# omerkurt-okt/buck-gnn

Measured on NVIDIA B200. Metric: graphs/sec, higher is better.
Workload: dtype f16

## Files before the change

buckgnn_b200/capi.py:

```python
from __future__ import annotations

import ctypes as C
import os
import threading

from .build import LIB_PATH as _DEFAULT_LIB_PATH

LIB_PATH = os.environ.get("BG_LIB_PATH", _DEFAULT_LIB_PATH)

BG_BF16, BG_F32, BG_F16 = 0, 1, 2
BG_AGGR_MEAN, BG_AGGR_SUM, BG_AGGR_MAX = 0, 1, 2
BG_BIG_ROW_THRESHOLD = 64
BG_MAX_GEMM_SEGMENTS = 8
ABI_VERSION = 11

AGGR_CODES = {"mean": BG_AGGR_MEAN, "sum": BG_AGGR_SUM, "add": BG_AGGR_SUM, "max": BG_AGGR_MAX}

EXPORTED_SYMBOLS = (
    "bg_abi_version", "bg_last_error", "bg_device_check", "bg_watchdog_info_host", "bg_set_sm_partition",
    "bg_csr_max_big_rows", "bg_csr_workspace_bytes", "bg_csr_build",
    "bg_batch_info", "bg_graph_ptr_build", "bg_publish_words", "bg_encoder_front",
    "bg_aggregate_workspace_bytes", "bg_hubfold_workspace_bytes", "bg_sage_aggregate", "bg_gemm512",
    "bg_sage_fused512", "bg_sage_aggregate_hubs", "bg_gemm128", "bg_gemm128_gathered", "bg_pool_head128", "bg_pool_head_blocks128",
    "bg_wgrad512", "bg_pool_workspace_bytes", "bg_pool_head", "bg_pool_block_flags", "bg_pool_head_blocks", "bg_cast_f32", "bg_split_tf32",
    "bg_expand_rowptr", "bg_add",
    "bg_train_workspace_bytes", "bg_bn_batch_stats", "bg_bn_act_forward", "bg_sage_backward_rows",
    "bg_transpose_chunks", "bg_mask_narrow", "bg_reduce_partials", "bg_colsum_workspace_bytes", "bg_colsum", "bg_pool_backward",
    "bg_sgemm_workspace_bytes", "bg_sgemm", "bg_eigen_loss", "bg_dropout_mask", "bg_collate_ptr", "bg_collate", "bg_expand_wire",
    "bg_dropout_residual", "bg_grad_mask", "bg_segment_expand",
    "bg_sag_workspace_bytes", "bg_sag_select", "bg_sag_connect", "bg_gather_rows", "bg_index_invert", "bg_index_gather",
    "bg_sag_pool_backward", "bg_max_aggregate_backward", "bg_max_bwd_workspace_bytes",
    "bg_bn_batch_stats128", "bg_bn_act_forward128", "bg_sage_backward_rows128", "bg_pool_backward128",
    "bg_max_aggregate_backward128", "bg_wgrad128",
    "bg_dropout_residual128", "bg_grad_mask128", "bg_segment_expand128", "bg_wgrad128_ld",
)


class BuckGNNError(RuntimeError):
    def __init__(self, status: int, where: str, message: str):
        super().__init__(f"{where} failed with status {status}: {message}")
        self.status = status


class GemmSegment(C.Structure):
    _fields_ = [("a", C.c_void_p), ("lda", C.c_int64), ("b", C.c_void_p), ("ldb", C.c_int64),
                ("k", C.c_int32), ("b_groups", C.c_int32)]


class Epilogue(C.Structure):
    _fields_ = [("bias_host", C.c_void_p), ("bn_scale_host", C.c_void_p), ("bn_shift_host", C.c_void_p),
                ("residual", C.c_void_p), ("ldr", C.c_int64), ("normalize", C.c_int32), ("relu", C.c_int32),
                ("gather", C.c_void_p * 2),
                ("gather_idx", C.c_void_p * 2), ("gather_ld", C.c_int64), ("inv_norm_out", C.c_void_p),
                ("pool_block_sums", C.c_void_p), ("pool_block_keep", C.c_void_p)]


class FusedAggregate(C.Structure):
    _fields_ = [("x", C.c_void_p), ("ldx", C.c_int64), ("rowptr", C.c_void_p), ("col", C.c_void_p),
                ("aggr", C.c_int32), ("n_big", C.c_int32), ("hub_agg", C.c_void_p), ("big_rows", C.c_void_p)]


_lib = None
_lock = threading.Lock()
_P, _I64, _I32, _SZP = C.c_void_p, C.c_int64, C.c_int32, C.POINTER(C.c_size_t)

_SIGNATURES = {
    "bg_abi_version": (C.c_int, []),
    "bg_last_error": (C.c_char_p, []),
    "bg_device_check": (C.c_int, []),
    "bg_watchdog_info_host": (C.c_int, [C.POINTER(C.c_uint32)]),
    "bg_set_sm_partition": (C.c_int, [C.c_int, C.c_int]),
    "bg_csr_max_big_rows": (_I64, [_I64]),
    "bg_csr_workspace_bytes": (C.c_int, [_I64, _I64, _SZP]),
    "bg_csr_build": (C.c_int, [_P, _I64, _I64, C.c_int, _P, _P, _P, _P, _P, _P, _P, _P, C.c_size_t, _P]),
    "bg_batch_info": (C.c_int, [_P, _I64, _P, _P]),
    "bg_publish_words": (C.c_int, [_P, _P, _I32, _P]),
    "bg_graph_ptr_build": (C.c_int, [_P, _I64, _I64, _P, _P]),
    "bg_encoder_front": (C.c_int, [_P, _I64, _I32, _P, _P, _P, _P, _P, _P, C.c_int, _P, _P]),
    "bg_expand_rowptr": (C.c_int, [_P, _I64, _I64, _P, _P, _P, C.c_int, C.c_int, _P]),
    "bg_add": (C.c_int, [_P, _P, _P, _P, C.c_int, _I64, _P]),
    "bg_aggregate_workspace_bytes": (C.c_int, [_I32, _SZP]),
    "bg_hubfold_workspace_bytes": (C.c_int, [_I64, C.c_int, _I32, _I32, _SZP]),
    "bg_sage_aggregate": (C.c_int, [_P, _P, C.c_int, _I64, _I32, _P, _P, _P, _I32, C.c_int, _P, _P, _I32, _P,
                                    C.c_size_t, _P]),
    "bg_gemm512": (C.c_int, [C.POINTER(GemmSegment), _I32, _I64, C.c_int, C.c_int, C.POINTER(Epilogue), _P,
                             C.c_int, _I64, C.c_int, _P]),
    "bg_sage_fused512": (C.c_int, [C.POINTER(GemmSegment), _I32, _I64, C.c_int, C.c_int, C.POINTER(Epilogue),
                                   C.POINTER(FusedAggregate), _P, C.c_int, _I64, _P]),
    "bg_sage_aggregate_hubs": (C.c_int, [_P, C.c_int, _P, _P, _P, _I32, C.c_int, _P, _P, C.c_size_t, _P]),
    "bg_gemm128": (C.c_int, [C.POINTER(GemmSegment), _I32, _I64, C.c_int, C.c_int, C.POINTER(Epilogue), _P,
                             C.c_int, _I64, C.c_int, _P]),
    "bg_gemm128_gathered": (C.c_int, [C.POINTER(GemmSegment), _I32, _I64, C.c_int, C.c_int, C.POINTER(Epilogue), _P,
                                      C.c_int, _I64, C.c_int, _P]),
    "bg_pool_head128": (C.c_int, [_P, C.c_int, _I64, _P, _I64, C.c_int, _P, _P, _P, _P, _P, _P, _P, _P, _I32, _P, _P,
                                  _P, C.c_size_t, _P, _P]),
    "bg_pool_head_blocks128": (C.c_int, [_P, C.c_int, _I64, _P, _I64, C.c_int, _P, _P, _P, _P, _P, _P, _P, _P, _I32, _P,
                                         _P, _P, _P, _P, C.c_size_t, _P, _P]),
    "bg_wgrad512": (C.c_int, [_P, _I64, _P, _I32, _I64, C.c_int, _I64, _I32, _I64, _P, _P]),
    "bg_pool_workspace_bytes": (C.c_int, [_I64, _SZP]),
    "bg_pool_head": (C.c_int, [_P, C.c_int, _I64, _P, _I64, C.c_int, _P, _P, _P, _P, _P, _P, _P, _P, _I32, _P, _P,
                               _P, C.c_size_t, _P, _P]),
    "bg_pool_block_flags": (C.c_int, [_P, _I64, _I64, _P, _P]),
    "bg_pool_head_blocks": (C.c_int, [_P, C.c_int, _I64, _P, _I64, C.c_int, _P, _P, _P, _P, _P, _P, _P, _P, _I32, _P, _P,
                                      _P, _P, _P, C.c_size_t, _P, _P]),
    "bg_cast_f32": (C.c_int, [_P, _P, C.c_int, _I64, _P]),
    "bg_split_tf32": (C.c_int, [_P, _P, _P, _I64, _P]),
    "bg_train_workspace_bytes": (C.c_int, [_I64, _SZP]),
# ... 84 lines not shown
    buf = (C.c_uint32 * 4)()
    _check(load().bg_watchdog_info_host(buf), "bg_watchdog_info_host")
    return list(buf)


def csr_max_big_rows(n_edges: int) -> int:
    return int(load().bg_csr_max_big_rows(n_edges))


def _query(fn_name: str, *args) -> int:
    out = C.c_size_t(0)
    _check(getattr(load(), fn_name)(*args, C.byref(out)), fn_name)
    return int(out.value)


def csr_workspace_bytes(n_nodes: int, n_edges: int) -> int:
    return _query("bg_csr_workspace_bytes", n_nodes, n_edges)


def aggregate_workspace_bytes(n_big: int) -> int:
    return _query("bg_aggregate_workspace_bytes", n_big)


def pool_workspace_bytes(n_graphs: int) -> int:
    return _query("bg_pool_workspace_bytes", n_graphs)


def csr_build(edge_index, n_edges, n_nodes, key_row, rowptr, col, perm, big_rows, info, ws, ws_bytes, stream,
              hub_lo=None, hub_of_row=None):
    _check(load().bg_csr_build(edge_index, n_edges, n_nodes, key_row, rowptr, col, perm, big_rows, info,
                               hub_lo, hub_of_row, ws, ws_bytes, stream), "bg_csr_build")


def batch_info(batch, n_nodes, info, stream):
    _check(load().bg_batch_info(batch, n_nodes, info, stream), "bg_batch_info")


def publish_words(src, dst_host_mapped, n, stream):
    _check(load().bg_publish_words(src, dst_host_mapped, n, stream), "bg_publish_words")


def graph_ptr_build(batch, n_nodes, n_graphs, graph_ptr, stream):
    _check(load().bg_graph_ptr_build(batch, n_nodes, n_graphs, graph_ptr, stream), "bg_graph_ptr_build")


def encoder_front(x, n_nodes, n_features, w1, b1, w2, b2, out, out_dtype, stream, row_gather=None, nonfinite=None):
    _check(load().bg_encoder_front(x, n_nodes, n_features, w1, b1, w2, b2, row_gather, out, out_dtype, nonfinite, stream),
           "bg_encoder_front")


def expand_rowptr(rowptr, n_rows, n_entries, row_of, iota, nonempty, nonempty_dtype, stream, as_count=False):
    _check(load().bg_expand_rowptr(rowptr, n_rows, n_entries, row_of, iota, nonempty, nonempty_dtype,
                                   int(bool(as_count)), stream), "bg_expand_rowptr")


def add(a, b, c, out, dtype, n, stream):
    _check(load().bg_add(a, b, c, out, dtype, n, stream), "bg_add")


def hubfold_workspace_bytes(n_nodes: int, dtype: int, n_big: int, hub_max_degree: int) -> int:
    return _query("bg_hubfold_workspace_bytes", n_nodes, dtype, n_big, hub_max_degree)


def sage_aggregate(x, out, dtype, n_nodes, rowptr, col, big_rows, n_big, aggr, ws, ws_bytes, stream, width=512,
                   hub_lo=None, hub_of_row=None, hub_max_degree=0):
    _check(load().bg_sage_aggregate(x, out, dtype, n_nodes, width, rowptr, col, big_rows, n_big, aggr,
# ... 267 lines not shown
```

buckgnn_b200/csrc/capi.cu:

```cuda
#include <cstdio>
#include <cstring>

#include "common.cuh"
#include "csr_build.cuh"
#include "aggregate.cuh"
#include "aggregate_window.cuh"
#include "encoder.cuh"
#include "gemm_tc.cuh"
#include "gemm128.cuh"
#include "pool_head.cuh"
#include "train.cuh"
#include "sag_pool.cuh"
#include "max_bwd.cuh"

namespace bg {

static thread_local char g_last_error[512] = "";

void set_last_cuda_error(cudaError_t e, const char* what, const char* file, int line) {
  snprintf(g_last_error, sizeof(g_last_error), "CUDA error %d (%s) at %s:%d: %s", (int)e,
           cudaGetErrorString(e), file, line, what);
}
static int fail(int code, const char* msg) {
  snprintf(g_last_error, sizeof(g_last_error), "%s", msg);
// ... 332 lines not shown
  const int max_big = (int)bg_csr_max_big_rows(E);
  const int sms = sm_count();
  BG_CUDA_OK(cudaMemsetAsync(w.deg, 0, sizeof(int32_t) * (size_t)(N + 1), stream));
  if ((hub_lo != nullptr) != (hub_of_row != nullptr)) return fail(BG_ERR_INVALID, "bg_csr_build: hub_lo and hub_of_row go together");
  BG_CUDA_OK(cudaMemsetAsync(info, 0, sizeof(int32_t) * 2, stream));
  BG_CUDA_OK(cudaMemsetAsync(info + 4, 0, sizeof(int32_t) * 3, stream));
  BG_CUDA_OK(cudaMemsetAsync(rowptr, 0, sizeof(int32_t), stream));
  if (hub_of_row && N > 0) BG_CUDA_OK(cudaMemsetAsync(hub_of_row, 0xff, sizeof(int32_t) * (size_t)N, stream));
  if (N == 0) return BG_OK;
  if (E > 0) {
    k_csr_hist<<<grid_for(E, 256, sms * 16), 256, 0, stream>>>(key, E, N, w.deg, info);
    BG_LAUNCH_OK();
  }
  k_scan_block_sums<<<w.n_scan_blocks, 1024, 0, stream>>>(w.deg, N, w.block_sums);
  BG_LAUNCH_OK();
  k_scan_of_sums<<<1, 1024, 0, stream>>>(w.block_sums, w.n_scan_blocks);
  BG_LAUNCH_OK();
  k_scan_apply<<<w.n_scan_blocks, 1024, 0, stream>>>(w.deg, N, w.block_sums, rowptr, w.cursor, big_rows, info, max_big);
  BG_LAUNCH_OK();
  if (E > 0) {
    k_csr_fill<<<grid_for(E, 256, sms * 16), 256, 0, stream>>>(key, E, N, w.cursor, perm);
    BG_LAUNCH_OK();
    k_csr_sort_small<<<(unsigned)ceil_div64(N, 256), 256, 0, stream>>>(rowptr, N, other, perm, col, info);
    BG_LAUNCH_OK();
    static bool attr_set = false;
    const int sort_smem = kSortSmemElems * (int)sizeof(int32_t);
    if (!attr_set) {
      BG_CUDA_OK(cudaFuncSetAttribute(k_csr_sort_big, cudaFuncAttributeMaxDynamicSharedMemorySize, sort_smem));
      attr_set = true;
    }
    k_csr_sort_big<<<sms, 1024, sort_smem, stream>>>(rowptr, big_rows, info, max_big, other, N, perm, col, hub_lo, hub_of_row);
    BG_LAUNCH_OK();
  }
  return BG_OK;
}

int bg_batch_info(const int64_t* batch, int64_t N, int32_t* info, void* stream_) {
  cudaStream_t stream = static_cast<cudaStream_t>(stream_);
  if (!info || N < 0 || (N > 0 && !batch)) return fail(BG_ERR_INVALID, "bg_batch_info: bad argument");
  BG_CUDA_OK(cudaMemsetAsync(info, 0, sizeof(int32_t) * 2, stream));
  if (N == 0) return BG_OK;
  k_batch_info<<<grid_for(N, 256, sm_count() * 8), 256, 0, stream>>>(batch, N, info);
  BG_LAUNCH_OK();
  return BG_OK;
}

int bg_graph_ptr_build(const int64_t* batch, int64_t N, int64_t G, int32_t* graph_ptr, void* stream_) {
  cudaStream_t stream = static_cast<cudaStream_t>(stream_);
  if (!graph_ptr || N < 0 || G < 0 || (N > 0 && !batch)) return fail(BG_ERR_INVALID, "bg_graph_ptr_build: bad argument");
  k_graph_ptr<<<grid_for(N + 1, 256, sm_count() * 8), 256, 0, stream>>>(batch, N, G, graph_ptr);
  BG_LAUNCH_OK();
  return BG_OK;
}

int bg_publish_words(const int32_t* src, int32_t* dst_host_mapped, int32_t n, void* stream_) {
  cudaStream_t stream = static_cast<cudaStream_t>(stream_);
  if (!src || !dst_host_mapped || n <= 0 || n > 256) return fail(BG_ERR_INVALID, "bg_publish_words: bad argument");
  k_publish_words<<<1, 256, 0, stream>>>(src, dst_host_mapped, n);
  BG_LAUNCH_OK();
  return BG_OK;
}

int bg_encoder_front(const float* x, int64_t N, int32_t F, const float* w1, const float* b1,
                     const float* w2, const float* b2, const int32_t* row_gather, void* out, int out_dtype,
                     int32_t* nonfinite_flag, void* stream_) {
  cudaStream_t stream = static_cast<cudaStream_t>(stream_);
// ... 1216 lines not shown
```

buckgnn_b200/csrc/csr_build.cuh:

```cuda
#pragma once
#include "common.cuh"

namespace bg {

constexpr int kScanItemsPerBlock = 4096;
constexpr int kSortSmemElems = 57344;

BG_DEVINL bool key_ok(int64_t k, int64_t N) { return k >= 0 && k < N; }
BG_DEVINL int32_t checked_col(int64_t o, int64_t N, int32_t* __restrict__ info) {
  if (o < 0 || o >= N) { atomicOr(&info[0], 1); return 0; }
  return (int32_t)o;
}

__global__ void k_csr_hist(const int64_t* __restrict__ key, int64_t E, int64_t N,
                           int32_t* __restrict__ deg, int32_t* __restrict__ info) {
  int64_t stride = (int64_t)gridDim.x * blockDim.x;
  bool bad = false;
  for (int64_t e = (int64_t)blockIdx.x * blockDim.x + threadIdx.x; e < E; e += stride) {
    int64_t k = key[e];
    if (!key_ok(k, N)) { bad = true; continue; }
    atomicAdd(&deg[k], 1);
  }
  if (bad) atomicOr(&info[0], 1);
}
// ... 186 lines not shown
                                                       const int64_t* __restrict__ other, int64_t N,
                                                       int32_t* __restrict__ perm, int32_t* __restrict__ col,
                                                       int32_t* __restrict__ hub_lo, int32_t* __restrict__ hub_of_row) {
  extern __shared__ int32_t sbuf[];
  int32_t n_big = min(info[1], max_big);
  for (int32_t b = blockIdx.x; b < n_big; b += gridDim.x) {
    const int32_t r = big_rows[b];
    const int32_t s = rowptr[r], n = rowptr[r + 1] - s;
    int32_t P = 1;
    while (P < n) P <<= 1;
    if (bitmap_sort_row(perm + s, n, reinterpret_cast<uint32_t*>(sbuf) + 64, sbuf)) {
      for (int32_t i = threadIdx.x; i < n; i += blockDim.x) col[s + i] = checked_col(other[perm[s + i]], N, info);
      __syncthreads();
    } else if (n <= kSortSmemElems) {
      for (int32_t i = threadIdx.x; i < n; i += blockDim.x) sbuf[i] = perm[s + i];
      __syncthreads();
      bitonic_ascending(sbuf, n, P);
      for (int32_t i = threadIdx.x; i < n; i += blockDim.x) {
        int32_t p = sbuf[i];
        perm[s + i] = p;
        col[s + i] = checked_col(other[p], N, info);
      }
      __syncthreads();
    } else {
      bitonic_ascending(perm + s, n, P);
      for (int32_t i = threadIdx.x; i < n; i += blockDim.x) col[s + i] = checked_col(other[perm[s + i]], N, info);
      __syncthreads();
    }
    if (hub_of_row) mark_range_hub(b, col + s, n, hub_lo, hub_of_row, info);
    __syncthreads();
  }
}

__global__ void k_batch_info(const int64_t* __restrict__ batch, int64_t N, int32_t* __restrict__ info) {
  int64_t stride = (int64_t)gridDim.x * blockDim.x;
  bool bad = false;
  for (int64_t i = (int64_t)blockIdx.x * blockDim.x + threadIdx.x; i < N; i += stride) {
    int64_t b = batch[i];
    if (b < 0 || b >= 0x7fffffffLL) bad = true;
    if (i > 0 && batch[i - 1] > b) bad = true;
    if (i == N - 1) info[0] = (int32_t)(b + 1);
  }
  if (bad) atomicOr(&info[1], 1);
}

__global__ void k_graph_ptr(const int64_t* __restrict__ batch, int64_t N, int64_t G,
                            int32_t* __restrict__ graph_ptr) {
  int64_t stride = (int64_t)gridDim.x * blockDim.x;
  for (int64_t i = (int64_t)blockIdx.x * blockDim.x + threadIdx.x; i <= N; i += stride) {
    int64_t prev = (i == 0) ? -1 : batch[i - 1];
    int64_t cur = (i == N) ? G : batch[i];
    if (cur > G) cur = G;
    for (int64_t g = prev + 1; g <= cur; ++g) graph_ptr[g] = (int32_t)i;
  }
}

struct CsrWorkspace {
  int32_t* deg;
  int32_t* cursor;
  int32_t* block_sums;
  int32_t n_scan_blocks;
  size_t bytes;
};

static inline CsrWorkspace csr_workspace_layout(void* base, int64_t N) {
  CsrWorkspace w;
// ... 16 lines not shown
```

buckgnn_b200/engine.py:

```python
from __future__ import annotations

import os
from dataclasses import dataclass
from typing import Dict, List, Optional, Tuple

import torch

from . import capi

_TORCH = {capi.BG_BF16: torch.bfloat16, capi.BG_F16: torch.float16, capi.BG_F32: torch.float32}
PRECISION_FORMATS = {
    "fp16": (capi.BG_F16, capi.BG_F16),
    "bf16": (capi.BG_BF16, capi.BG_BF16),
    "tf32": (capi.BG_F32, capi.BG_F32),
    "fp32": (capi.BG_F32, capi.BG_F32),
}
PRECISIONS = tuple(PRECISION_FORMATS)


def default_precision(aggr: str) -> str:
    return "fp16" if aggr in ("mean", "max") else "tf32"


def _stream() -> int:
# ... 22 lines not shown
            if self.pushed:
                torch.cuda.nvtx.range_push(self.name)
            if self.owner.enabled:
                self.e0 = torch.cuda.Event(enable_timing=True)
                self.e1 = torch.cuda.Event(enable_timing=True)
                self.e0.record()
            return self

        def __exit__(self, *a):
            if self.owner.enabled:
                self.e1.record()
                self.owner.spans.append((self.name, self.e0, self.e1))
            if self.pushed:
                torch.cuda.nvtx.range_pop()

    def span(self, name):
        return self._Span(self, name)

    def summary(self):
        torch.cuda.synchronize()
        out = {}
        for name, e0, e1 in self.spans:
            ms, n = out.get(name, (0.0, 0))
            out[name] = (ms + e0.elapsed_time(e1), n + 1)
        return out


TIMERS = _KernelTimers()


def LAUNCHES_PER_FORWARD(num_layers: int, folded: bool = True, fused_pool: bool = False) -> int:
    extra = 1 if fused_pool else 0
    if folded:
        return 7 + 3 + 1 + 3 * num_layers + 2 + extra
    return 7 + 3 + 2 + 3 * num_layers + 2 + extra


def _p(t: Optional[torch.Tensor]) -> Optional[int]:
    return None if t is None else t.data_ptr()


def _require_cuda(t: torch.Tensor, name: str) -> None:
    if not t.is_cuda:
        raise RuntimeError(f"buckgnn_b200: `{name}` must be a CUDA tensor (got {t.device}); the hot path has "
                           "no CPU implementation")


@dataclass
class GraphIndex:
    n_nodes: int
    n_edges: int
    rowptr: torch.Tensor
    col: torch.Tensor
    perm: torch.Tensor
    big_rows: torch.Tensor
    n_big: int
    graph_ptr: torch.Tensor
    n_graphs: int
    hub_lo: Optional[torch.Tensor] = None
    hub_of_row: Optional[torch.Tensor] = None
    hub_max_degree: int = 0
    has_empty_rows: bool = True


class PendingGraphIndex:

    def __init__(self, edge_index, batch, n_nodes, key_row):
        _require_cuda(edge_index, "edge_index")
        if edge_index.dtype != torch.int64 or edge_index.dim() != 2 or edge_index.shape[0] != 2:
            raise ValueError("edge_index must be an int64 tensor of shape [2, E]")
        self.edge_index = edge_index.contiguous()
        dev = edge_index.device
        self.E, self.N = edge_index.shape[1], int(n_nodes)
        E, N = self.E, self.N
        s = _stream()
        i32 = dict(dtype=torch.int32, device=dev)
        self.rowptr = torch.empty(N + 1, **i32)
        self.col = torch.empty(max(E, 1), **i32)
        self.perm = torch.empty(max(E, 1), **i32)
        self.big_rows = torch.empty(capi.csr_max_big_rows(E), **i32)
        self.hub_lo = torch.empty(capi.csr_max_big_rows(E), **i32)
        self.hub_of_row = torch.empty(max(N, 1), **i32)
        self.info = torch.zeros(8, **i32)
        ws_bytes = capi.csr_workspace_bytes(N, E)
        self._ws = torch.empty(ws_bytes, dtype=torch.uint8, device=dev)
        with TIMERS.span("csr_build"):
            capi.csr_build(self.edge_index.data_ptr(), E, N, key_row, self.rowptr.data_ptr(), self.col.data_ptr(),
                           self.perm.data_ptr(), self.big_rows.data_ptr(), self.info.data_ptr(),
                           self._ws.data_ptr(), ws_bytes, s, hub_lo=self.hub_lo.data_ptr(),
                           hub_of_row=self.hub_of_row.data_ptr())
        self.batch = None
        if batch is not None:
            _require_cuda(batch, "batch")
            if batch.dtype != torch.int64 or batch.dim() != 1 or batch.shape[0] != N:
                raise ValueError("batch must be an int64 tensor of shape [N]")
            self.batch = batch.contiguous()
            capi.batch_info(self.batch.data_ptr(), N, self.info[2:].data_ptr(), s)
        self._host = torch.zeros(8, dtype=torch.int32).pin_memory()
        capi.publish_words(self.info.data_ptr(), self._host.data_ptr(), 8, s)
        self._done = torch.cuda.Event()
        self._done.record()

    def finish(self) -> "GraphIndex":
        self._done.synchronize()
        host = self._host.tolist()
        N, E = self.N, self.E
        i32 = dict(dtype=torch.int32, device=self.edge_index.device)
        if host[0] & 1:
            raise IndexError("edge_index contains node ids outside [0, num_nodes)")
        n_big = host[1]
        if self.batch is None:
            n_graphs = 1
            graph_ptr = torch.tensor([0, N], **i32)
        else:
            if host[3]:
                raise ValueError("buckgnn_b200 needs a sorted, non-negative `batch` vector (PyG DataLoader order)")
            n_graphs = host[2] if N > 0 else 0
            graph_ptr = torch.empty(n_graphs + 1, **i32)
            capi.graph_ptr_build(self.batch.data_ptr(), N, n_graphs, graph_ptr.data_ptr(), _stream())
        ranges = n_big > 0 and host[4] == 0
        return GraphIndex(N, E, self.rowptr, self.col, self.perm, self.big_rows, n_big, graph_ptr, n_graphs,
                          hub_lo=self.hub_lo if ranges else None, hub_of_row=self.hub_of_row if ranges else None,
                          hub_max_degree=host[5] if ranges else 0, has_empty_rows=bool(host[6]) or N == 0)


def begin_graph_index(edge_index: torch.Tensor, batch: Optional[torch.Tensor], n_nodes: int,
                      key_row: int = 1) -> PendingGraphIndex:
    return PendingGraphIndex(edge_index, batch, n_nodes, key_row)


def build_graph_index(edge_index: torch.Tensor, batch: Optional[torch.Tensor], n_nodes: int,
                      key_row: int = 1) -> GraphIndex:
    return begin_graph_index(edge_index, batch, n_nodes, key_row).finish()


@dataclass
class LinearPack:
    k: int
    parts: Tuple[torch.Tensor, ...]
    code: int = capi.BG_F32


def pack_linear(weight: torch.Tensor, precision: str) -> LinearPack:
    w = weight.detach().to(torch.float32).contiguous()
    k = w.shape[1]
    s = _stream()
    code = PRECISION_FORMATS[precision][1]
    if code != capi.BG_F32:
        out = torch.empty(w.shape, dtype=_TORCH[code], device=w.device)
        capi.cast_f32(w.data_ptr(), out.data_ptr(), code, w.numel(), s)
        return LinearPack(k, (out,), code)
    if precision == "tf32":
# ... 492 lines not shown
```

include/buckgnn_b200.h:

```cpp
#ifndef BUCKGNN_B200_H_
#define BUCKGNN_B200_H_

#include <stddef.h>
#include <stdint.h>

#ifdef __cplusplus
extern "C" {
#endif

#define BG_ABI_VERSION 11

typedef enum bg_status {
  BG_OK = 0,
  BG_ERR_INVALID = -1,
  BG_ERR_CUDA = -2,
  BG_ERR_WORKSPACE = -3,
  BG_ERR_UNSUPPORTED = -4,
  BG_ERR_DEVICE = -5
} bg_status;

typedef enum bg_dtype { BG_BF16 = 0, BG_F32 = 1, BG_F16 = 2 } bg_dtype;

typedef enum bg_aggr { BG_AGGR_MEAN = 0, BG_AGGR_SUM = 1, BG_AGGR_MAX = 2 } bg_aggr;

int bg_abi_version(void);
const char* bg_last_error(void);
int bg_device_check(void);
int bg_watchdog_info_host(uint32_t* out4_host);
int bg_set_sm_partition(int gemm_sms, int agg_sms);

#define BG_BIG_ROW_THRESHOLD 64
int64_t bg_csr_max_big_rows(int64_t n_edges);
int bg_csr_workspace_bytes(int64_t n_nodes, int64_t n_edges, size_t* bytes_host);
int bg_csr_build(const int64_t* edge_index, int64_t n_edges, int64_t n_nodes, int key_row,
                 int32_t* rowptr, int32_t* col, int32_t* perm, int32_t* big_rows, int32_t* info,
                 int32_t* hub_lo, int32_t* hub_of_row,
                 void* workspace, size_t workspace_bytes, void* stream);

int bg_batch_info(const int64_t* batch, int64_t n_nodes, int32_t* info, void* stream);
int bg_publish_words(const int32_t* src, int32_t* dst_host_mapped, int32_t n, void* stream);
int bg_graph_ptr_build(const int64_t* batch, int64_t n_nodes, int64_t n_graphs, int32_t* graph_ptr,
                       void* stream);

int bg_encoder_front(const float* x, int64_t n_nodes, int32_t n_features,
                     const float* w1, const float* b1, const float* w2, const float* b2,
                     const int32_t* row_gather, void* out, int out_dtype, int32_t* nonfinite_flag, void* stream);

int bg_aggregate_workspace_bytes(int32_t n_big, size_t* bytes_host);
int bg_hubfold_workspace_bytes(int64_t n_nodes, int dtype, int32_t n_big, int32_t hub_max_degree,
                               size_t* bytes_host);
int bg_sage_aggregate(const void* x, void* out, int dtype, int64_t n_nodes, int32_t width,
                      const int32_t* rowptr, const int32_t* col,
                      const int32_t* big_rows, int32_t n_big, int aggr,
                      const int32_t* hub_lo, const int32_t* hub_of_row, int32_t hub_max_degree,
                      void* workspace, size_t workspace_bytes, void* stream);

#define BG_MAX_GEMM_SEGMENTS 8
typedef struct bg_gemm_segment {
  const void* a; int64_t lda;
  const void* b; int64_t ldb;
  int32_t k;
  int32_t b_groups;
} bg_gemm_segment;

typedef struct bg_epilogue {
  const float* bias_host;
  const float* bn_scale_host;
  const float* bn_shift_host;
  const void* residual;
  int64_t ldr;
// ... 188 lines not shown
```

Baseline: 30030.

## Build CSR per graph in a single fused kernel with fallback to general path

```diff
diff --git a/buckgnn_b200/capi.py b/buckgnn_b200/capi.py
--- a/buckgnn_b200/capi.py
+++ b/buckgnn_b200/capi.py
@@ -12,13 +12,14 @@
 BG_AGGR_MEAN, BG_AGGR_SUM, BG_AGGR_MAX = 0, 1, 2
 BG_BIG_ROW_THRESHOLD = 64
 BG_MAX_GEMM_SEGMENTS = 8
+CSR_GROUPED_CAPACITY = 57344
 ABI_VERSION = 11
 
 AGGR_CODES = {"mean": BG_AGGR_MEAN, "sum": BG_AGGR_SUM, "add": BG_AGGR_SUM, "max": BG_AGGR_MAX}
 
 EXPORTED_SYMBOLS = (
     "bg_abi_version", "bg_last_error", "bg_device_check", "bg_watchdog_info_host", "bg_set_sm_partition",
-    "bg_csr_max_big_rows", "bg_csr_workspace_bytes", "bg_csr_build",
+    "bg_csr_max_big_rows", "bg_csr_workspace_bytes", "bg_csr_build", "bg_csr_build_grouped",
     "bg_batch_info", "bg_graph_ptr_build", "bg_publish_words", "bg_encoder_front",
     "bg_aggregate_workspace_bytes", "bg_hubfold_workspace_bytes", "bg_sage_aggregate", "bg_gemm512",
     "bg_sage_fused512", "bg_sage_aggregate_hubs", "bg_gemm128", "bg_gemm128_gathered", "bg_pool_head128", "bg_pool_head_blocks128",
@@ -73,6 +74,7 @@
     "bg_csr_max_big_rows": (_I64, [_I64]),
     "bg_csr_workspace_bytes": (C.c_int, [_I64, _I64, _SZP]),
     "bg_csr_build": (C.c_int, [_P, _I64, _I64, C.c_int, _P, _P, _P, _P, _P, _P, _P, _P, C.c_size_t, _P]),
+    "bg_csr_build_grouped": (C.c_int, [_P, _I64, _I64, C.c_int, _P, _P, _P, _P, _P, _P, _P, _P, _P, _P]),
     "bg_batch_info": (C.c_int, [_P, _I64, _P, _P]),
     "bg_publish_words": (C.c_int, [_P, _P, _I32, _P]),
     "bg_graph_ptr_build": (C.c_int, [_P, _I64, _I64, _P, _P]),
@@ -223,6 +225,12 @@
                                hub_lo, hub_of_row, ws, ws_bytes, stream), "bg_csr_build")
 
 
+def csr_build_grouped(edge_index, n_edges, n_nodes, key_row, batch, n_graphs_word, rowptr, col, perm, big_rows, info,
+                      hub_lo, hub_of_row, stream):
+    _check(load().bg_csr_build_grouped(edge_index, n_edges, n_nodes, key_row, batch, n_graphs_word, rowptr, col, perm,
+                                       big_rows, info, hub_lo, hub_of_row, stream), "bg_csr_build_grouped")
+
+
 def batch_info(batch, n_nodes, info, stream):
     _check(load().bg_batch_info(batch, n_nodes, info, stream), "bg_batch_info")
 
diff --git a/buckgnn_b200/csrc/capi.cu b/buckgnn_b200/csrc/capi.cu
--- a/buckgnn_b200/csrc/capi.cu
+++ b/buckgnn_b200/csrc/capi.cu
@@ -388,6 +388,37 @@
     k_csr_sort_big<<<sms, 1024, sort_smem, stream>>>(rowptr, big_rows, info, max_big, other, N, perm, col, hub_lo, hub_of_row);
     BG_LAUNCH_OK();
   }
+  return BG_OK;
+}
+
+int bg_csr_build_grouped(const int64_t* edge_index, int64_t E, int64_t N, int key_row,
+                         const int64_t* batch, const int32_t* n_graphs_word,
+                         int32_t* rowptr, int32_t* col, int32_t* perm, int32_t* big_rows, int32_t* info,
+                         int32_t* hub_lo, int32_t* hub_of_row, void* stream_) {
+  cudaStream_t stream = static_cast<cudaStream_t>(stream_);
+  if (E < 0 || N < 0 || E >= 0x7fffffffLL || N >= 0x7fffffffLL)
+    return fail(BG_ERR_INVALID, "bg_csr_build_grouped: sizes out of range");
+  if (key_row != 0 && key_row != 1) return fail(BG_ERR_INVALID, "bg_csr_build_grouped: key_row must be 0 or 1");
+  if (!rowptr || !info || (E > 0 && (!edge_index || !col || !perm || !big_rows)) || (N > 0 && (!hub_lo || !hub_of_row)))
+    return fail(BG_ERR_INVALID, "bg_csr_build_grouped: null pointer");
+  if ((batch != nullptr) != (n_graphs_word != nullptr))
+    return fail(BG_ERR_INVALID, "bg_csr_build_grouped: batch and n_graphs_word go together");
+  BG_CUDA_OK(cudaMemsetAsync(info, 0, sizeof(int32_t) * 2, stream));
+  BG_CUDA_OK(cudaMemsetAsync(info + 4, 0, sizeof(int32_t) * 4, stream));
+  BG_CUDA_OK(cudaMemsetAsync(rowptr, 0, sizeof(int32_t), stream));
+  if (N == 0) return BG_OK;
+  const int64_t* key = edge_index + (size_t)key_row * E;
+  const int64_t* other = edge_index + (size_t)(1 - key_row) * E;
+  static bool attr_set = false;
+  const int smem = kSortSmemElems * (int)sizeof(int32_t);
+  if (!attr_set) {
+    BG_CUDA_OK(cudaFuncSetAttribute(k_csr_grouped, cudaFuncAttributeMaxDynamicSharedMemorySize, smem));
+    attr_set = true;
+  }
+  k_csr_grouped<<<sm_count(), kGroupedThreads, smem, stream>>>(key, other, E, N, batch, n_graphs_word, rowptr, col, perm,
+                                                                big_rows, info, (int32_t)bg_csr_max_big_rows(E), hub_lo,
+                                                                hub_of_row);
+  BG_LAUNCH_OK();
   return BG_OK;
 }
 
diff --git a/buckgnn_b200/csrc/csr_build.cuh b/buckgnn_b200/csrc/csr_build.cuh
--- a/buckgnn_b200/csrc/csr_build.cuh
+++ b/buckgnn_b200/csrc/csr_build.cuh
@@ -242,6 +242,180 @@
   }
 }
 
+constexpr int kGroupedThreads = 1024;
+constexpr int kGroupedUnroll = 4;
+
+BG_DEVINL int64_t grouped_smem_words(int64_t n, int64_t m) {
+  return n + m + ((m + 31) >> 5) + 2 * (m / (kBigRowThreshold + 1) + 1);
+}
+
+template <class P0, class P1>
+BG_DEVINL void cta_lower_bound2(int64_t n, P0 p0, P1 p1, int64_t& r0, int64_t& r1, int64_t* s_res ) {
+  const int32_t T = (int32_t)blockDim.x >> 1;
+  const int half = (int32_t)threadIdx.x >= T;
+  const int32_t j = (int32_t)threadIdx.x - half * T;
+  int64_t lo = 0, hi = n;
+  while (!__syncthreads_and(lo == hi)) {
+    const int64_t len = hi - lo;
+    const int64_t step = (len + T - 1) / T;
+    const int64_t nb = len > 0 ? (len + step - 1) / step : 0;
+    bool f = false;
+    if (j < nb) {
+      const int64_t q = min(lo + (j + 1) * step, hi) - 1;
+      f = half ? !p1(q) : !p0(q);
+    }
+    const int64_t c0 = __syncthreads_count(f && !half), c1 = __syncthreads_count(f && half);
+    const int64_t c = half ? c1 : c0;
+    if (len > 0) {
+      const int64_t nlo = min(lo + c * step, hi);
+      hi = c < nb ? min(lo + (c + 1) * step, hi) - 1 : hi;
+      lo = nlo;
+    }
+  }
+  if (threadIdx.x == 0) s_res[0] = lo;
+  if (threadIdx.x == (unsigned)T) s_res[1] = lo;
+  __syncthreads();
+  r0 = s_res[0];
+  r1 = s_res[1];
+  __syncthreads();
+}
+
+__global__ void __launch_bounds__(kGroupedThreads) k_csr_grouped(
+    const int64_t* __restrict__ key, const int64_t* __restrict__ other, int64_t E, int64_t N,
+    const int64_t* __restrict__ batch, const int32_t* __restrict__ n_graphs_word,
+    int32_t* __restrict__ rowptr, int32_t* __restrict__ col, int32_t* __restrict__ perm,
+    int32_t* __restrict__ big_rows, int32_t* __restrict__ info, int32_t max_big,
+    int32_t* __restrict__ hub_lo, int32_t* __restrict__ hub_of_row) {
+  extern __shared__ int32_t pool[];
+  __shared__ int32_t red[64];
+  __shared__ int64_t s_res[2];
+  __shared__ int32_t s_nbig;
+  const int64_t G = batch ? (int64_t)n_graphs_word[0] : 1;
+  if (G < 1 || G > N) {
+    if (blockIdx.x == 0 && threadIdx.x == 0) atomicOr(&info[7], 1);
+    return;
+  }
+  for (int64_t g = blockIdx.x; g < G; g += gridDim.x) {
+    int64_t n0 = 0, n1 = N, e0, e1;
+    if (batch) cta_lower_bound2(N, [&](int64_t i) { return batch[i] >= g; },
+                                   [&](int64_t i) { return batch[i] >= g + 1; }, n0, n1, s_res);
+    cta_lower_bound2(E, [&](int64_t i) { return key[i] >= n0; }, [&](int64_t i) { return key[i] >= n1; }, e0, e1, s_res);
+    const int64_t n = n1 - n0, m = e1 - e0;
+    if (n <= 0 || m < 0 || (n0 == 0 && e0 != 0) || (n1 == N && e1 != E) || n > kSortSmemElems || m > kSortSmemElems ||
+        grouped_smem_words(n, m) > kSortSmemElems) {
+      if (threadIdx.x == 0) atomicOr(&info[7], 1);
+      continue;
+    }
+    int32_t* cnt = pool;
+    int32_t* sperm = cnt + n;
+    uint32_t* bits = reinterpret_cast<uint32_t*>(sperm + m);
+    int32_t* hubs = sperm + m + ((m + 31) >> 5);
+    for (int64_t j = threadIdx.x; j < n; j += blockDim.x) { cnt[j] = 0; hub_of_row[n0 + j] = -1; }
+    if (threadIdx.x == 0) s_nbig = 0;
+    __syncthreads();
+
+    int bad = 0;
+    for (int64_t b = threadIdx.x; b < m; b += kGroupedUnroll * (int64_t)blockDim.x) {
+      int64_t k[kGroupedUnroll], o[kGroupedUnroll];
+#pragma unroll
+      for (int u = 0; u < kGroupedUnroll; ++u) {
+        const int64_t i = b + u * (int64_t)blockDim.x;
+        k[u] = i < m ? key[e0 + i] : n0;
+        o[u] = i < m ? other[e0 + i] : n0;
+      }
+#pragma unroll
+      for (int u = 0; u < kGroupedUnroll; ++u) {
+        if (b + u * (int64_t)blockDim.x >= m) continue;
+        if (k[u] < n0 || k[u] >= n1 || o[u] < n0 || o[u] >= n1) { bad = 1; continue; }
+        atomicAdd(&cnt[k[u] - n0], 1);
+      }
+    }
+    if (__syncthreads_or(bad)) {
+      if (threadIdx.x == 0) atomicOr(&info[7], 1);
+      continue;
+    }
+
+    const int32_t per = (int32_t)((n + blockDim.x - 1) / blockDim.x);
+    const int32_t j0 = (int32_t)min(n, (int64_t)threadIdx.x * per), j1 = (int32_t)min(n, (int64_t)j0 + per);
+    int32_t mine = 0;
+    for (int32_t j = j0; j < j1; ++j) mine += cnt[j];
+    int32_t total;
+    int32_t run = block_exclusive_scan(mine, red, total);
+    int empty_row = 0;
+    for (int32_t j = j0; j < j1; ++j) {
+      const int32_t d = cnt[j];
+      cnt[j] = run;
+      rowptr[n0 + j] = (int32_t)e0 + run;
+      if (d > kBigRowThreshold) {
+        const int32_t slot = atomicAdd(&info[1], 1);
+        if (slot < max_big) big_rows[slot] = (int32_t)(n0 + j);
+        atomicMax(&info[5], d);
+        const int32_t l = atomicAdd(&s_nbig, 1);
+        hubs[2 * l] = j;
+        hubs[2 * l + 1] = slot;
+      }
+      empty_row |= d == 0;
+      run += d;
+    }
+    if (n1 == N && threadIdx.x == 0) rowptr[N] = (int32_t)E;
+    if (__syncthreads_or(empty_row) && threadIdx.x == 0) atomicOr(&info[6], 1);
+
+    for (int64_t b = threadIdx.x; b < m; b += kGroupedUnroll * (int64_t)blockDim.x) {
+      int64_t k[kGroupedUnroll];
+#pragma unroll
+      for (int u = 0; u < kGroupedUnroll; ++u) {
+        const int64_t i = b + u * (int64_t)blockDim.x;
+        k[u] = i < m ? key[e0 + i] : n0;
+      }
+#pragma unroll
+      for (int u = 0; u < kGroupedUnroll; ++u) {
+        const int64_t i = b + u * (int64_t)blockDim.x;
+        if (i < m) sperm[atomicAdd(&cnt[k[u] - n0], 1)] = (int32_t)i;
+      }
+    }
+    __syncthreads();
+
+    for (int64_t j = threadIdx.x; j < n; j += blockDim.x) {
+      const int32_t s = j ? cnt[j - 1] : 0, e = cnt[j];
+      if (e - s > kBigRowThreshold) continue;
+      for (int32_t i = s + 1; i < e; ++i) {
+        const int32_t v = sperm[i];
+        int32_t q = i - 1;
+        while (q >= s && sperm[q] > v) { sperm[q + 1] = sperm[q]; --q; }
+        sperm[q + 1] = v;
+      }
+    }
+    __syncthreads();
+    const int32_t n_hub = s_nbig;
+    for (int32_t l = 0; l < n_hub; ++l) {
+      const int32_t j = hubs[2 * l], s = j ? cnt[j - 1] : 0;
+      bitmap_sort_row(sperm + s, cnt[j] - s, bits, red);
+    }
+
+    for (int64_t b = threadIdx.x; b < m; b += kGroupedUnroll * (int64_t)blockDim.x) {
+      int32_t p[kGroupedUnroll];
+      int64_t o[kGroupedUnroll];
+#pragma unroll
+      for (int u = 0; u < kGroupedUnroll; ++u) {
+        const int64_t i = b + u * (int64_t)blockDim.x;
+        p[u] = i < m ? sperm[i] : 0;
+        o[u] = i < m ? other[e0 + p[u]] : 0;
+      }
+#pragma unroll
+      for (int u = 0; u < kGroupedUnroll; ++u) {
+        const int64_t i = b + u * (int64_t)blockDim.x;
+        if (i < m) { perm[e0 + i] = (int32_t)e0 + p[u]; col[e0 + i] = (int32_t)o[u]; }
+      }
+    }
+    __syncthreads();
+    for (int32_t l = 0; l < n_hub; ++l) {
+      const int32_t j = hubs[2 * l], slot = hubs[2 * l + 1], s = j ? cnt[j - 1] : 0;
+      if (slot < max_big) mark_range_hub(slot, col + e0 + s, cnt[j] - s, hub_lo, hub_of_row, info);
+      __syncthreads();
+    }
+  }
+}
+
 __global__ void k_batch_info(const int64_t* __restrict__ batch, int64_t N, int32_t* __restrict__ info) {
   int64_t stride = (int64_t)gridDim.x * blockDim.x;
   bool bad = false;
diff --git a/buckgnn_b200/engine.py b/buckgnn_b200/engine.py
--- a/buckgnn_b200/engine.py
+++ b/buckgnn_b200/engine.py
@@ -78,8 +78,8 @@
 def LAUNCHES_PER_FORWARD(num_layers: int, folded: bool = True, fused_pool: bool = False) -> int:
     extra = 1 if fused_pool else 0
     if folded:
-        return 7 + 3 + 1 + 3 * num_layers + 2 + extra
-    return 7 + 3 + 2 + 3 * num_layers + 2 + extra
+        return 1 + 3 + 1 + 3 * num_layers + 2 + extra
+    return 1 + 3 + 2 + 3 * num_layers + 2 + extra
 
 
 def _p(t: Optional[torch.Tensor]) -> Optional[int]:
@@ -128,20 +128,36 @@
         self.hub_lo = torch.empty(capi.csr_max_big_rows(E), **i32)
         self.hub_of_row = torch.empty(max(N, 1), **i32)
         self.info = torch.zeros(8, **i32)
-        ws_bytes = capi.csr_workspace_bytes(N, E)
-        self._ws = torch.empty(ws_bytes, dtype=torch.uint8, device=dev)
-        with TIMERS.span("csr_build"):
-            capi.csr_build(self.edge_index.data_ptr(), E, N, key_row, self.rowptr.data_ptr(), self.col.data_ptr(),
-                           self.perm.data_ptr(), self.big_rows.data_ptr(), self.info.data_ptr(),
-                           self._ws.data_ptr(), ws_bytes, s, hub_lo=self.hub_lo.data_ptr(),
-                           hub_of_row=self.hub_of_row.data_ptr())
+        self.key_row = key_row
         self.batch = None
         if batch is not None:
             _require_cuda(batch, "batch")
             if batch.dtype != torch.int64 or batch.dim() != 1 or batch.shape[0] != N:
                 raise ValueError("batch must be an int64 tensor of shape [N]")
             self.batch = batch.contiguous()
-            capi.batch_info(self.batch.data_ptr(), N, self.info[2:].data_ptr(), s)
+        self.grouped = self.batch is not None or N + E <= capi.CSR_GROUPED_CAPACITY
+        with TIMERS.span("csr_build"):
+            if self.batch is not None:
+                capi.batch_info(self.batch.data_ptr(), N, self.info[2:].data_ptr(), s)
+            if self.grouped:
+                capi.csr_build_grouped(self.edge_index.data_ptr(), E, N, key_row, _p(self.batch),
+                                       None if self.batch is None else self.info[2:].data_ptr(),
+                                       self.rowptr.data_ptr(), self.col.data_ptr(), self.perm.data_ptr(),
+                                       self.big_rows.data_ptr(), self.info.data_ptr(), self.hub_lo.data_ptr(),
+                                       self.hub_of_row.data_ptr(), s)
+            else:
+                self._build_general(s)
+        self._publish(s)
+
+    def _build_general(self, s):
+        ws_bytes = capi.csr_workspace_bytes(self.N, self.E)
+        self._ws = torch.empty(ws_bytes, dtype=torch.uint8, device=self.edge_index.device)
+        capi.csr_build(self.edge_index.data_ptr(), self.E, self.N, self.key_row, self.rowptr.data_ptr(),
+                       self.col.data_ptr(), self.perm.data_ptr(), self.big_rows.data_ptr(), self.info.data_ptr(),
+                       self._ws.data_ptr(), ws_bytes, s, hub_lo=self.hub_lo.data_ptr(),
+                       hub_of_row=self.hub_of_row.data_ptr())
+
+    def _publish(self, s):
         self._host = torch.zeros(8, dtype=torch.int32).pin_memory()
         capi.publish_words(self.info.data_ptr(), self._host.data_ptr(), 8, s)
         self._done = torch.cuda.Event()
@@ -150,6 +166,13 @@
     def finish(self) -> "GraphIndex":
         self._done.synchronize()
         host = self._host.tolist()
+        if self.grouped and host[7]:
+            self.grouped = False
+            s = _stream()
+            self._build_general(s)
+            self._publish(s)
+            self._done.synchronize()
+            host = self._host.tolist()
         N, E = self.N, self.E
         i32 = dict(dtype=torch.int32, device=self.edge_index.device)
         if host[0] & 1:
diff --git a/include/buckgnn_b200.h b/include/buckgnn_b200.h
--- a/include/buckgnn_b200.h
+++ b/include/buckgnn_b200.h
@@ -36,6 +36,10 @@
                  int32_t* rowptr, int32_t* col, int32_t* perm, int32_t* big_rows, int32_t* info,
                  int32_t* hub_lo, int32_t* hub_of_row,
                  void* workspace, size_t workspace_bytes, void* stream);
+int bg_csr_build_grouped(const int64_t* edge_index, int64_t n_edges, int64_t n_nodes, int key_row,
+                         const int64_t* batch, const int32_t* n_graphs_word,
+                         int32_t* rowptr, int32_t* col, int32_t* perm, int32_t* big_rows, int32_t* info,
+                         int32_t* hub_lo, int32_t* hub_of_row, void* stream);
 
 int bg_batch_info(const int64_t* batch, int64_t n_nodes, int32_t* info, void* stream);
 int bg_publish_words(const int32_t* src, int32_t* dst_host_mapped, int32_t n, void* stream);
```

Measured after the change: 30150, median of 6. About the same (+0.4%).

## Build CSR per graph in shared memory when batch vector is given

Applied to the files above, without the earlier changes.

```diff
diff --git a/buckgnn_b200/capi.py b/buckgnn_b200/capi.py
--- a/buckgnn_b200/capi.py
+++ b/buckgnn_b200/capi.py
@@ -18,7 +18,7 @@
 
 EXPORTED_SYMBOLS = (
     "bg_abi_version", "bg_last_error", "bg_device_check", "bg_watchdog_info_host", "bg_set_sm_partition",
-    "bg_csr_max_big_rows", "bg_csr_workspace_bytes", "bg_csr_build",
+    "bg_csr_max_big_rows", "bg_csr_workspace_bytes", "bg_csr_build", "bg_csr_build_graphs",
     "bg_batch_info", "bg_graph_ptr_build", "bg_publish_words", "bg_encoder_front",
     "bg_aggregate_workspace_bytes", "bg_hubfold_workspace_bytes", "bg_sage_aggregate", "bg_gemm512",
     "bg_sage_fused512", "bg_sage_aggregate_hubs", "bg_gemm128", "bg_gemm128_gathered", "bg_pool_head128", "bg_pool_head_blocks128",
@@ -73,6 +73,7 @@
     "bg_csr_max_big_rows": (_I64, [_I64]),
     "bg_csr_workspace_bytes": (C.c_int, [_I64, _I64, _SZP]),
     "bg_csr_build": (C.c_int, [_P, _I64, _I64, C.c_int, _P, _P, _P, _P, _P, _P, _P, _P, C.c_size_t, _P]),
+    "bg_csr_build_graphs": (C.c_int, [_P, _I64, _I64, C.c_int, _P, _P, _P, _P, _P, _P, _P, _P, _P, _P, C.c_size_t, _P]),
     "bg_batch_info": (C.c_int, [_P, _I64, _P, _P]),
     "bg_publish_words": (C.c_int, [_P, _P, _I32, _P]),
     "bg_graph_ptr_build": (C.c_int, [_P, _I64, _I64, _P, _P]),
@@ -223,6 +224,12 @@
                                hub_lo, hub_of_row, ws, ws_bytes, stream), "bg_csr_build")
 
 
+def csr_build_graphs(edge_index, n_edges, n_nodes, key_row, batch, rowptr, col, perm, big_rows, info, hub_lo, hub_of_row,
+                     graph_ptr, ws, ws_bytes, stream):
+    _check(load().bg_csr_build_graphs(edge_index, n_edges, n_nodes, key_row, batch, rowptr, col, perm, big_rows, info,
+                                      hub_lo, hub_of_row, graph_ptr, ws, ws_bytes, stream), "bg_csr_build_graphs")
+
+
 def batch_info(batch, n_nodes, info, stream):
     _check(load().bg_batch_info(batch, n_nodes, info, stream), "bg_batch_info")
 
diff --git a/buckgnn_b200/csrc/capi.cu b/buckgnn_b200/csrc/capi.cu
--- a/buckgnn_b200/csrc/capi.cu
+++ b/buckgnn_b200/csrc/capi.cu
@@ -388,6 +388,39 @@
     k_csr_sort_big<<<sms, 1024, sort_smem, stream>>>(rowptr, big_rows, info, max_big, other, N, perm, col, hub_lo, hub_of_row);
     BG_LAUNCH_OK();
   }
+  return BG_OK;
+}
+
+int bg_csr_build_graphs(const int64_t* edge_index, int64_t E, int64_t N, int key_row, const int64_t* batch,
+                        int32_t* rowptr, int32_t* col, int32_t* perm, int32_t* big_rows, int32_t* info,
+                        int32_t* hub_lo, int32_t* hub_of_row, int32_t* graph_ptr,
+                        void* workspace, size_t workspace_bytes, void* stream_) {
+  cudaStream_t stream = static_cast<cudaStream_t>(stream_);
+  if (E <= 0 || N <= 0 || E >= 0x7fffffffLL || N >= 0x7fffffffLL)
+    return fail(BG_ERR_INVALID, "bg_csr_build_graphs: sizes out of range (E and N must be positive)");
+  if (key_row != 0 && key_row != 1) return fail(BG_ERR_INVALID, "bg_csr_build_graphs: key_row must be 0 or 1");
+  if (!edge_index || !batch || !rowptr || !col || !perm || !big_rows || !info || !graph_ptr || !workspace)
+    return fail(BG_ERR_INVALID, "bg_csr_build_graphs: null pointer");
+  if ((hub_lo != nullptr) != (hub_of_row != nullptr)) return fail(BG_ERR_INVALID, "bg_csr_build_graphs: hub_lo and hub_of_row go together");
+  CsrWorkspace w = csr_workspace_layout(workspace, N);
+  if (workspace_bytes < w.bytes) return fail(BG_ERR_WORKSPACE, "bg_csr_build_graphs: workspace too small");
+  const int64_t* key = edge_index + (size_t)key_row * E;
+  const int64_t* other = edge_index + (size_t)(1 - key_row) * E;
+  const int sms = sm_count();
+  BG_CUDA_OK(cudaMemsetAsync(info, 0, sizeof(int32_t) * 2, stream));
+  BG_CUDA_OK(cudaMemsetAsync(info + 4, 0, sizeof(int32_t) * 4, stream));
+  if (hub_of_row) BG_CUDA_OK(cudaMemsetAsync(hub_of_row, 0xff, sizeof(int32_t) * (size_t)N, stream));
+  k_csr_graph_ranges<<<grid_for((N > E ? N : E) + 1, 256, sms * 16), 256, 0, stream>>>(key, E, batch, N, graph_ptr, w.deg, info);
+  BG_LAUNCH_OK();
+  static bool attr_set = false;
+  if (!attr_set) {
+    BG_CUDA_OK(cudaFuncSetAttribute(k_csr_graphs, cudaFuncAttributeMaxDynamicSharedMemorySize, kGraphSmemBytes));
+    attr_set = true;
+  }
+  k_csr_graphs<<<2 * sms, kGraphThreads, kGraphSmemBytes, stream>>>(key, other, batch, N, graph_ptr, w.deg, rowptr, col, perm,
+                                                                    big_rows, info, (int32_t)bg_csr_max_big_rows(E),
+                                                                    hub_lo, hub_of_row);
+  BG_LAUNCH_OK();
   return BG_OK;
 }
 
diff --git a/buckgnn_b200/csrc/csr_build.cuh b/buckgnn_b200/csrc/csr_build.cuh
--- a/buckgnn_b200/csrc/csr_build.cuh
+++ b/buckgnn_b200/csrc/csr_build.cuh
@@ -242,6 +242,157 @@
   }
 }
 
+constexpr int kGraphThreads = 1024;
+constexpr int kUnroll = 4;
+constexpr int kRegSort = 8;
+constexpr int kGraphRowCap = 12288;
+constexpr int kGraphEdgeCap = 131072;
+constexpr int kGraphBigCap = kGraphEdgeCap / (kBigRowThreshold + 1) + 1;
+constexpr int kGraphSmemBytes = (int)sizeof(int32_t) * ((kGraphRowCap + 1) + 2 * kGraphBigCap + 64 + kGraphEdgeCap / 32);
+
+__global__ void k_csr_graph_ranges(const int64_t* __restrict__ key, int64_t E, const int64_t* __restrict__ batch, int64_t N,
+                                   int32_t* __restrict__ graph_ptr, int32_t* __restrict__ edge_ptr, int32_t* __restrict__ info) {
+  const int64_t last = batch[N - 1];
+  const int64_t G = (last >= 0 && last < N) ? last + 1 : N;
+  auto graph_of_edge = [&](int64_t e) -> int64_t {
+    const int64_t k = key[e];
+    return key_ok(k, N) ? batch[k] : -2;
+  };
+  const int64_t stride = (int64_t)gridDim.x * blockDim.x;
+  bool bad = false;
+  for (int64_t i = (int64_t)blockIdx.x * blockDim.x + threadIdx.x; i <= max(N, E); i += stride) {
+    if (i <= N) {
+      const int64_t prev = (i == 0) ? -1 : batch[i - 1];
+      const int64_t cur = (i == N) ? G : batch[i];
+      if (i < N && (cur < 0 || cur >= N || prev > cur)) bad = true;
+      for (int64_t g = max(prev + 1, (int64_t)0); g <= min(cur, N); ++g) graph_ptr[g] = (int32_t)i;
+    }
+    if (i <= E) {
+      const int64_t prev = (i == 0) ? -1 : graph_of_edge(i - 1);
+      const int64_t cur = (i == E) ? G : graph_of_edge(i);
+      if (i < E && (cur < 0 || prev > cur)) bad = true;
+      for (int64_t g = max(prev + 1, (int64_t)0); g <= min(cur, N); ++g) edge_ptr[g] = (int32_t)i;
+    }
+  }
+  if (bad) atomicOr(&info[7], 1);
+}
+
+__global__ void __launch_bounds__(kGraphThreads) k_csr_graphs(const int64_t* __restrict__ key, const int64_t* __restrict__ other,
+                                                              const int64_t* __restrict__ batch, int64_t N,
+                                                              const int32_t* __restrict__ graph_ptr, const int32_t* __restrict__ edge_ptr,
+                                                              int32_t* __restrict__ rowptr, int32_t* __restrict__ col,
+                                                              int32_t* __restrict__ perm, int32_t* __restrict__ big_rows,
+                                                              int32_t* __restrict__ info, int32_t max_big,
+                                                              int32_t* __restrict__ hub_lo, int32_t* __restrict__ hub_of_row) {
+  extern __shared__ int32_t smem[];
+  int32_t* cnt = smem;
+  int32_t* big = cnt + kGraphRowCap + 1;
+  int32_t* red = big + 2 * kGraphBigCap;
+  uint32_t* bits = reinterpret_cast<uint32_t*>(red + 64);
+  __shared__ int32_t n_big_s, broken_s;
+  if (threadIdx.x == 0) broken_s = *reinterpret_cast<volatile int32_t*>(info + 7);
+  __syncthreads();
+  if (broken_s) return;
+  const int64_t G = batch[N - 1] + 1;
+  const int tid = threadIdx.x, nt = blockDim.x;
+  for (int64_t g = blockIdx.x; g < G; g += gridDim.x) {
+    const int32_t r0 = graph_ptr[g], nr = graph_ptr[g + 1] - r0;
+    const int32_t e0 = edge_ptr[g], ne = edge_ptr[g + 1] - e0;
+    if (nr > kGraphRowCap || ne > kGraphEdgeCap) {
+      if (tid == 0) atomicOr(&info[7], 1);
+      continue;
+    }
+    for (int32_t i = tid; i < nr; i += nt) cnt[i] = 0;
+    if (tid == 0) n_big_s = 0;
+    __syncthreads();
+    for (int64_t base = e0 + tid; base < e0 + ne; base += kUnroll * nt) {
+      int64_t k[kUnroll];
+#pragma unroll
+      for (int u = 0; u < kUnroll; ++u) k[u] = (base + u * nt < e0 + ne) ? key[base + u * nt] : -1;
+#pragma unroll
+      for (int u = 0; u < kUnroll; ++u) if (k[u] >= 0) atomicAdd(&cnt[k[u] - r0], 1);
+    }
+    __syncthreads();
+    const int32_t per = (nr + nt - 1) / nt;
+    const int32_t a = min(nr, tid * per), b = min(nr, a + per);
+    int32_t mine = 0;
+    for (int32_t i = a; i < b; ++i) mine += cnt[i];
+    int32_t total;
+    int32_t run = block_exclusive_scan(mine, red, total);
+    for (int32_t i = a; i < b; ++i) {
+      const int32_t d = cnt[i];
+      rowptr[r0 + i] = e0 + run;
+      cnt[i] = run;
+      if (d > kBigRowThreshold) {
+        const int32_t slot = atomicAdd(&info[1], 1);
+        atomicMax(&info[5], d);
+        if (slot < max_big) {
+          big_rows[slot] = r0 + i;
+          const int32_t l = atomicAdd(&n_big_s, 1);
+          big[2 * l] = i;
+          big[2 * l + 1] = slot;
+        }
+      }
+      if (d == 0) atomicOr(&info[6], 1);
+      run += d;
+    }
+    if (g == G - 1 && tid == 0) rowptr[N] = e0 + ne;
+    __syncthreads();
+    for (int64_t base = e0 + tid; base < e0 + ne; base += kUnroll * nt) {
+      int64_t k[kUnroll];
+#pragma unroll
+      for (int u = 0; u < kUnroll; ++u) k[u] = (base + u * nt < e0 + ne) ? key[base + u * nt] : -1;
+#pragma unroll
+      for (int u = 0; u < kUnroll; ++u)
+        if (k[u] >= 0) perm[e0 + atomicAdd(&cnt[k[u] - r0], 1)] = (int32_t)(base + u * nt);
+    }
+    __syncthreads();
+    for (int32_t i = tid; i < nr; i += nt) {
+      const int32_t s = e0 + (i ? cnt[i - 1] : 0), t = e0 + cnt[i];
+      if (t - s > kBigRowThreshold) continue;
+      if (t - s <= kRegSort) {
+        int32_t v[kRegSort];
+        int64_t o[kRegSort];
+#pragma unroll
+        for (int u = 0; u < kRegSort; ++u) v[u] = (u < t - s) ? perm[s + u] : 0x7fffffff;
+#pragma unroll
+        for (int p = 0; p < kRegSort; ++p) {
+#pragma unroll
+          for (int u = p & 1; u + 1 < kRegSort; u += 2) {
+            const int32_t x = min(v[u], v[u + 1]), y = max(v[u], v[u + 1]);
+            v[u] = x;
+            v[u + 1] = y;
+          }
+        }
+#pragma unroll
+        for (int u = 0; u < kRegSort; ++u) o[u] = (u < t - s) ? other[v[u]] : 0;
+#pragma unroll
+        for (int u = 0; u < kRegSort; ++u)
+          if (u < t - s) { perm[s + u] = v[u]; col[s + u] = checked_col(o[u], N, info); }
+        continue;
+      }
+      for (int32_t j = s + 1; j < t; ++j) {
+        const int32_t v = perm[j];
+        int32_t k = j - 1;
+        while (k >= s && perm[k] > v) { perm[k + 1] = perm[k]; --k; }
+        perm[k + 1] = v;
+      }
+      for (int32_t j = s; j < t; ++j) col[j] = checked_col(other[perm[j]], N, info);
+    }
+    const int32_t nb = n_big_s;
+    for (int32_t l = 0; l < nb; ++l) {
+      const int32_t i = big[2 * l], slot = big[2 * l + 1];
+      const int32_t s = e0 + (i ? cnt[i - 1] : 0), n = e0 + cnt[i] - s;
+      bitmap_sort_row(perm + s, n, bits, red);
+      for (int32_t j = tid; j < n; j += nt) col[s + j] = checked_col(other[perm[s + j]], N, info);
+      __syncthreads();
+      if (hub_of_row) mark_range_hub(slot, col + s, n, hub_lo, hub_of_row, info);
+      __syncthreads();
+    }
+    __syncthreads();
+  }
+}
+
 __global__ void k_batch_info(const int64_t* __restrict__ batch, int64_t N, int32_t* __restrict__ info) {
   int64_t stride = (int64_t)gridDim.x * blockDim.x;
   bool bad = false;
diff --git a/buckgnn_b200/engine.py b/buckgnn_b200/engine.py
--- a/buckgnn_b200/engine.py
+++ b/buckgnn_b200/engine.py
@@ -78,8 +78,8 @@
 def LAUNCHES_PER_FORWARD(num_layers: int, folded: bool = True, fused_pool: bool = False) -> int:
     extra = 1 if fused_pool else 0
     if folded:
-        return 7 + 3 + 1 + 3 * num_layers + 2 + extra
-    return 7 + 3 + 2 + 3 * num_layers + 2 + extra
+        return 2 + 2 + 1 + 3 * num_layers + 2 + extra
+    return 2 + 2 + 2 + 3 * num_layers + 2 + extra
 
 
 def _p(t: Optional[torch.Tensor]) -> Optional[int]:
@@ -107,6 +107,9 @@
     hub_of_row: Optional[torch.Tensor] = None
     hub_max_degree: int = 0
     has_empty_rows: bool = True
+
+
+PER_GRAPH_CSR = True
 
 
 class PendingGraphIndex:
@@ -128,28 +131,51 @@
         self.hub_lo = torch.empty(capi.csr_max_big_rows(E), **i32)
         self.hub_of_row = torch.empty(max(N, 1), **i32)
         self.info = torch.zeros(8, **i32)
-        ws_bytes = capi.csr_workspace_bytes(N, E)
-        self._ws = torch.empty(ws_bytes, dtype=torch.uint8, device=dev)
-        with TIMERS.span("csr_build"):
-            capi.csr_build(self.edge_index.data_ptr(), E, N, key_row, self.rowptr.data_ptr(), self.col.data_ptr(),
-                           self.perm.data_ptr(), self.big_rows.data_ptr(), self.info.data_ptr(),
-                           self._ws.data_ptr(), ws_bytes, s, hub_lo=self.hub_lo.data_ptr(),
-                           hub_of_row=self.hub_of_row.data_ptr())
+        self._ws_bytes = capi.csr_workspace_bytes(N, E)
+        self._ws = torch.empty(self._ws_bytes, dtype=torch.uint8, device=dev)
+        self.key_row = key_row
         self.batch = None
         if batch is not None:
             _require_cuda(batch, "batch")
             if batch.dtype != torch.int64 or batch.dim() != 1 or batch.shape[0] != N:
                 raise ValueError("batch must be an int64 tensor of shape [N]")
             self.batch = batch.contiguous()
+        self._graph_ptr = None
+        with TIMERS.span("csr_build"):
+            if PER_GRAPH_CSR and self.batch is not None and N > 0 and E > 0:
+                self._graph_ptr = torch.empty(N + 1, **i32)
+                capi.csr_build_graphs(self.edge_index.data_ptr(), E, N, key_row, self.batch.data_ptr(),
+                                      self.rowptr.data_ptr(), self.col.data_ptr(), self.perm.data_ptr(),
+                                      self.big_rows.data_ptr(), self.info.data_ptr(), self.hub_lo.data_ptr(),
+                                      self.hub_of_row.data_ptr(), self._graph_ptr.data_ptr(), self._ws.data_ptr(),
+                                      self._ws_bytes, s)
+            else:
+                self._generic_build()
+        if self.batch is not None:
             capi.batch_info(self.batch.data_ptr(), N, self.info[2:].data_ptr(), s)
         self._host = torch.zeros(8, dtype=torch.int32).pin_memory()
-        capi.publish_words(self.info.data_ptr(), self._host.data_ptr(), 8, s)
+        self._publish()
+
+    def _generic_build(self):
+        capi.csr_build(self.edge_index.data_ptr(), self.E, self.N, self.key_row, self.rowptr.data_ptr(),
+                       self.col.data_ptr(), self.perm.data_ptr(), self.big_rows.data_ptr(), self.info.data_ptr(),
+                       self._ws.data_ptr(), self._ws_bytes, _stream(), hub_lo=self.hub_lo.data_ptr(),
+                       hub_of_row=self.hub_of_row.data_ptr())
+
+    def _publish(self):
+        capi.publish_words(self.info.data_ptr(), self._host.data_ptr(), 8, _stream())
         self._done = torch.cuda.Event()
         self._done.record()
 
     def finish(self) -> "GraphIndex":
         self._done.synchronize()
         host = self._host.tolist()
+        if self._graph_ptr is not None and host[7]:
+            self._graph_ptr = None
+            self._generic_build()
+            self._publish()
+            self._done.synchronize()
+            host = self._host.tolist()
         N, E = self.N, self.E
         i32 = dict(dtype=torch.int32, device=self.edge_index.device)
         if host[0] & 1:
@@ -162,8 +188,11 @@
             if host[3]:
                 raise ValueError("buckgnn_b200 needs a sorted, non-negative `batch` vector (PyG DataLoader order)")
             n_graphs = host[2] if N > 0 else 0
-            graph_ptr = torch.empty(n_graphs + 1, **i32)
-            capi.graph_ptr_build(self.batch.data_ptr(), N, n_graphs, graph_ptr.data_ptr(), _stream())
+            if self._graph_ptr is not None:
+                graph_ptr = self._graph_ptr[:n_graphs + 1]
+            else:
+                graph_ptr = torch.empty(n_graphs + 1, **i32)
+                capi.graph_ptr_build(self.batch.data_ptr(), N, n_graphs, graph_ptr.data_ptr(), _stream())
         ranges = n_big > 0 and host[4] == 0
         return GraphIndex(N, E, self.rowptr, self.col, self.perm, self.big_rows, n_big, graph_ptr, n_graphs,
                           hub_lo=self.hub_lo if ranges else None, hub_of_row=self.hub_of_row if ranges else None,
diff --git a/include/buckgnn_b200.h b/include/buckgnn_b200.h
--- a/include/buckgnn_b200.h
+++ b/include/buckgnn_b200.h
@@ -36,6 +36,10 @@
                  int32_t* rowptr, int32_t* col, int32_t* perm, int32_t* big_rows, int32_t* info,
                  int32_t* hub_lo, int32_t* hub_of_row,
                  void* workspace, size_t workspace_bytes, void* stream);
+int bg_csr_build_graphs(const int64_t* edge_index, int64_t n_edges, int64_t n_nodes, int key_row, const int64_t* batch,
+                        int32_t* rowptr, int32_t* col, int32_t* perm, int32_t* big_rows, int32_t* info,
+                        int32_t* hub_lo, int32_t* hub_of_row, int32_t* graph_ptr,
+                        void* workspace, size_t workspace_bytes, void* stream);
 
 int bg_batch_info(const int64_t* batch, int64_t n_nodes, int32_t* info, void* stream);
 int bg_publish_words(const int32_t* src, int32_t* dst_host_mapped, int32_t n, void* stream);
```

Measured after the change: 29490 before, 29790 after (median of 6 runs). Within noise of the previous version (+1.0%).
